# yalue/cudabrot

Measured on AMD Instinct MI355X. Metric: Msamples/sec (escaping points) + HBM GB/s, 4096x4096 max_iter=20000, 1/2/4/8 GPU, higher is better.
Workload: dtype f64

## Files before the change

cudabrot_amd/csrc/draw_wide.hip:

```cpp
#include <stdlib.h>

#include "draw_common.h"

#ifdef CB_BURNING_SHIP
#define CB_LAUNCH_NAME launch_draw_wide_ship
#else
#define CB_LAUNCH_NAME launch_draw_wide
#endif

namespace cb {

namespace {

constexpr int kWavesPerBlock = 4;
constexpr int kSlots = 4;
constexpr int kQ0Cap = 128;
constexpr int kQ1Cap = 96;
constexpr int kQ2Cap = 320;
constexpr int kHeadSteps = 4;
constexpr int kQ1Low = 32;
constexpr int kReplayMin = 56;
constexpr uint32_t kReplayBurst = 32;
constexpr int kPrioBehind = 2;
constexpr int kPrioAhead = 1;
constexpr uint32_t kBrentBits = 2;
constexpr uint32_t kPrioChunks = 64;
constexpr uint32_t kPrioHalves = 256;

static_assert(kQ0Cap >= 63 + 64, "Q0 must hold a full HEAD half-pass on top of 63 queued survivors");
static_assert(kQ1Cap >= kQ1Low - 1 + 64, "Q1 must hold a full MID pass on top of kQ1Low - 1 queued orbits");
static_assert(kQ2Cap >= 63 + 64 * kSlots, "Q2 must hold every orbit slot of a chunk on top of 63 queued points");

struct WideQueues {
  double q0_cr[kQ0Cap], q0_ci[kQ0Cap];
  double q1_cr[kQ1Cap], q1_ci[kQ1Cap], q1_r[kQ1Cap], q1_i[kQ1Cap];
  double q2_cr[kQ2Cap], q2_ci[kQ2Cap];
};
constexpr uint32_t kWideQueueWords = sizeof(WideQueues) / 8;
constexpr uint32_t kWideLanePlanes = kSlots * 6 + 2 + 4 + 1;
constexpr uint32_t kWidePlanesFront = (kCarryWordsPerWave - kCarryHeaderWords - kWideQueueWords) / 64;
__host__ __device__ constexpr uint32_t wide_plane(uint32_t p) {
  return p < kWidePlanesFront ? kCarryHeaderWords + kWideQueueWords + 64u * p
                              : kCarryWordsPerWave + kCarryHeaderWords + 64u * (p - kWidePlanesFront);
}
static_assert(kCarryHeaderWords + kWideQueueWords <= kCarryWordsPerWave, "the queues end in front of the second header");
// ... 643 lines not shown
  "v_cmpx_gt_u32_e32 vcc, %[nn], %[pidx]\n\t"    \
  "v_add_u32 %[pidx], %[q2h], %[pidx]\n\t"       \
  "v_subrev_u32 %[e], 320, %[pidx]\n\t"                   \
  "v_min_u32 %[pidx], %[pidx], %[e]\n\t"                  \
  "v_lshl_add_u32 %[pidx], %[pidx], 3, %[q2]\n\t"         \
  "ds_read_b64 %[cr], %[pidx]\n\t"                        \
  "ds_read_b64 %[ci], %[pidx] offset:2560\n\t"            \
  "s_or_b64 %[act], %[act], exec\n\t"                     \
  "v_mov_b32 %[pst], %[clk]\n\t"                          \
  "s_waitcnt lgkmcnt(0)\n\t"                              \
  "v_mul_f64 %[a], %[ci], %[ci]\n\t"             \
  "v_fma_f64 %[a], %[cr], %[cr], -%[a]\n\t"               \
  "v_fma_f64 %[i], " CB_AL "%[cr]" CB_AR ", " CB_AL "%[ci]" CB_AR ", %[ci]\n\t" \
  "v_fma_f64 %[r], %[a], 0.5, %[cr]\n\t"                  \
  "6:\n\t"                                                \
  "s_bcnt1_i32_b64 %[t], %[act]\n\t"                      \
  "s_cmp_eq_u32 %[t], 0\n\t"                              \
  "s_cbranch_scc1 2f\n\t"                                 \
  "s_sub_u32 %[ctr], %[q2c], %[nn]\n\t"          \
  "s_cmp_lg_u32 %[ctr], 0\n\t"                          \
  "s_cselect_b32 %[ctr], 1, %[minact]\n\t"              \
  "s_cmp_ge_u32 %[t], %[ctr]\n\t"                       \
  "s_cbranch_scc0 2f\n\t"
#define CBW_REPLAY_HEAD                                   \
  "s_sub_u32 %[ctr], %[n], 1\n\t"        \
  "s_mov_b32 %[ch], %[fill]\n\t"         \
  "s_mov_b64 exec, %[act]\n\t"                            \
  "v_mul_f64 %[a], %[r], %[r]\n\t"       \
  "v_fma_f64 %[a], %[i], %[i], %[a]\n\t"                  \
  "s_cmp_lg_u32 %[direct], 0\n\t"                         \
  "s_cbranch_scc1 7f\n\t"                                 \
  "1:\n\t"                                                \
  "s_bcnt1_i32_b64 %[t], %[act]\n\t"
#define CBW_REPLAY_STEP_COMMON                            \
  "s_add_u32 %[cs], %[cs], %[t]\n\t"                      \
  "v_cmp_nlt_f64_e64 %[alive], %[k16], %[a]\n\t"          \
  "v_mul_f64 %[a], %[i], %[i]\n\t"                        \
  "v_cmp_gt_u64_e64 %[hx], %[wb], %[fx]\n\t"              \
  "v_fma_f64 %[a], %[r], %[r], -%[a]\n\t"                 \
  "v_cmp_gt_u64_e64 vcc, %[hb], %[fy]\n\t"                \
  "v_fma_f64 %[i], " CB_AL "%[r]" CB_AR ", " CB_AL "%[i]" CB_AR ", %[ci]\n\t" \
  "v_cvt_i32_f64 %[col], %[fx]\n\t"                       \
  "v_fma_f64 %[r], %[a], 0.5, %[cr]\n\t"                  \
  "v_cvt_i32_f64 %[row], %[fy]\n\t"
#define CBW_REPLAY_LOOP                                   \
  CBW_REPLAY_STEP_COMMON                                  \
  "s_and_b64 vcc, vcc, %[hx]\n\t"                         \
  "v_mul_f64 %[a], %[r], %[r]\n\t"                        \
  "v_lshl_or_b32 %[e], %[row], 16, %[col]\n\t"            \
  "v_mbcnt_lo_u32_b32 %[pidx], vcc_lo, 0\n\t"             \
  "v_fma_f64 %[a], %[i], %[i], %[a]\n\t"                  \
  "v_mbcnt_hi_u32_b32 %[pidx], vcc_hi, %[pidx]\n\t"       \
  "s_bcnt1_i32_b64 %[t], vcc\n\t"                         \
  "v_add_lshl_u32 %[pidx], %[pidx], %[fill], 2\n\t"       \
  "s_and_b64 %[act], %[act], %[alive]\n\t"                \
  "s_mov_b64 exec, vcc\n\t"                               \
  "global_store_dword %[pidx], %[e], %[base]\n\t"         \
  "s_add_u32 %[fill], %[fill], %[t]\n\t"                  \
  "s_mov_b64 exec, %[act]\n\t"                            \
  "s_cbranch_execz 8f\n\t"               \
  "s_sub_u32 %[ctr], %[ctr], 1\n\t"      \
  "s_cbranch_scc0 1b\n\t"                                 \
  "s_add_u32 %[clk], %[clk], %[n]\n\t"   \
  "s_branch 18f\n\t"                                      \
  "8:\n\t"                                                \
  "s_sub_u32 %[t], %[n], %[ctr]\n\t"     \
  "s_add_u32 %[clk], %[clk], %[t]\n\t"                    \
  "18:\n\t"                                               \
  "s_sub_u32 %[ch], %[fill], %[ch]\n\t"
#define CBW_REPLAY_LOOP_CHUNKED                           \
  "s_add_u32 %[cs], %[cs], %[t]\n\t"                      \
  "v_cmp_nlt_f64_e64 %[alive], %[k16], %[a]\n\t"          \
  "v_cmp_gt_u64_e64 %[hx], %[wb], %[fx]\n\t"              \
  "v_cmp_gt_u64_e64 vcc, %[hb], %[fy]\n\t"                \
  "v_cvt_i32_f64 %[col], %[fx]\n\t"                       \
  "v_cvt_i32_f64 %[row], %[fy]\n\t"                       \
  "v_mul_f64 %[a], %[i], %[i]\n\t"                        \
  "v_mov_b32 %[lim], 1\n\t"                               \
  "s_and_b64 vcc, vcc, %[hx]\n\t"                         \
  "v_lshl_or_b32 %[e], %[row], 16, %[col]\n\t"            \
  "s_mov_b64 %[hit], vcc\n\t"                             \
  "s_mov_b64 exec, vcc\n\t"                               \
  "v_lshrrev_b32 %[row], 7, %[row]\n\t"                   \
  "v_lshrrev_b32 %[col], 7, %[col]\n\t"                   \
  "v_mad_u32_u24 %[row], %[row], %[tlx], %[col]\n\t"      \
  "v_lshrrev_b32 %[pidx], 10, %[row]\n\t"                 \
  "v_lshl_add_u32 %[col], %[pidx], 3, %[gcl]\n\t"         \
  "ds_add_rtn_u32 %[pos], %[col], %[lim]\n\t"             \
  "ds_read_b32 %[lim], %[col] offset:4\n\t"               \
  "s_bcnt1_i32_b64 %[t], vcc\n\t"                         \
  "s_mov_b64 exec, %[act]\n\t"                            \
  "v_fma_f64 %[a], %[r], %[r], -%[a]\n\t"                 \
// ... 53 lines not shown
  "s_add_u32 %[clk], %[clk], %[t]\n\t"                    \
  "9:\n\t"
#define CBW_REPLAY_END                                    \
  "2:\n\t"                                                \
  "s_mov_b64 exec, %[save]\n\t"                           \
  "s_nop 4\n\t"

struct ChunkOverflow {
  unsigned long long over;
  uint32_t word, group, pos, lim;
};
template <bool kPow2, bool kChunked>
__device__ __forceinline__ uint32_t replay_stage(uint32_t enable, unsigned long long &act, uint32_t q2_head,
                                                 uint32_t q2_count, uint32_t q2_lds, uint32_t min_active,
                                                 uint32_t n_steps, uint32_t direct, Orbit &p, uint32_t &p_start,
                                                 uint32_t *region, uint32_t &fill, uint32_t &clock,
                                                 uint32_t &lane_steps, uint32_t &hits, uint32_t cursors_lds,
                                                 ChunkOverflow &ovf) {
  static_assert(kQ2Cap == 320, "ring length and plane distance in CBW_REPLAY_REFILL");
  unsigned long long save, alive, hx, scp;
  uint32_t cs, ch, ctr, t, nn;
  double a, fx, fy, d0, d1, d2, d3, ox, oy;
  uint32_t pidx, e, col, row;
  unsigned long long over = 0ull, hit;
  uint32_t pos = 0u, lim = 0u;
  const uint32_t tlx = kChunked ? kernel_args()->bin.tiles_x : 0u;
  cursors_lds = __builtin_amdgcn_readfirstlane(cursors_lds);
  const KernelArgs ka = kernel_args();
  const double wb = ka->replay_bound_w, hb = ka->replay_bound_h;
  const uint32_t wi = (uint32_t) ka->w;
  const unsigned long long hist = reinterpret_cast<unsigned long long>(ka->hist);
  region = reinterpret_cast<uint32_t *>(uniform_u64(reinterpret_cast<unsigned long long>(region)));
  enable = __builtin_amdgcn_readfirstlane(enable);
  act = uniform_u64(act);
  fill = __builtin_amdgcn_readfirstlane(fill);
  clock = __builtin_amdgcn_readfirstlane(clock);
  n_steps = __builtin_amdgcn_readfirstlane(n_steps);
  q2_head = __builtin_amdgcn_readfirstlane(q2_head);
  q2_count = __builtin_amdgcn_readfirstlane(q2_count);
  min_active = __builtin_amdgcn_readfirstlane(min_active);
  direct = __builtin_amdgcn_readfirstlane(direct);
  const double k16 = 16.0;
  const double sx = ka->replay_scale_real, sy = ka->replay_scale_imag;
  const double oxs = ka->replay_offset_real, oys = ka->replay_offset_imag;
#define CBW_REPLAY_OUT                                                                                             \
  [r] "+v"(p.r), [i] "+v"(p.i), [cr] "+v"(p.cr), [ci] "+v"(p.ci), [pst] "+v"(p_start), [act] "+s"(act),            \
      [fill] "+s"(fill), [clk] "+s"(clock), [save] "=&s"(save), [alive] "=&s"(alive), [hx] "=&s"(hx),              \
      [cs] "=&s"(cs), [ch] "=&s"(ch), [ctr] "=&s"(ctr), [t] "=&s"(t), [nn] "=&s"(nn), [a] "=&v"(a), [fx] "=&v"(fx), \
      [fy] "=&v"(fy), [e] "=&v"(e), [col] "=&v"(col), [row] "=&v"(row), [pidx] "=&v"(pidx)
#define CBW_REPLAY_IN                                                                                              \
  [en] "s"(enable), [n] "s"(n_steps), [q2h] "s"(q2_head), [q2c] "s"(q2_count), [q2] "s"(q2_lds),                   \
      [minact] "s"(min_active), [direct] "s"(direct), [sx] "s"(sx), [sy] "s"(sy), [wb] "s"(wb), [hb] "s"(hb),      \
      [wi] "s"(wi), [hist] "s"(hist), [base] "s"(region), [k16] "s"(k16)
  (void) ox;
  (void) oy;
#define CBW_CHUNKED_OUT [over] "+s"(over), [hit] "=&s"(hit), [pos] "+v"(pos), [lim] "+v"(lim)
#define CBW_CHUNKED_IN [tlx] "s"(tlx), [gcl] "s"(cursors_lds)
  if (kPow2 && kChunked) {
    asm volatile("v_mov_b64 %[ox], %[oxs]\n\t"
                 "v_mov_b64 %[oy], %[oys]\n\t"
                 CBW_REPLAY_REFILL CBW_REPLAY_HEAD CBW_REPLAY_BIN_POW2 CBW_REPLAY_LOOP_CHUNKED
                 CBW_REPLAY_DIRECT(CBW_REPLAY_BIN_POW2) CBW_REPLAY_END
                 : CBW_REPLAY_OUT, [ox] "=&v"(ox), [oy] "=&v"(oy), CBW_CHUNKED_OUT
                 : CBW_REPLAY_IN, [oxs] "s"(oxs), [oys] "s"(oys), CBW_CHUNKED_IN
                 : "vcc", "scc", "memory");
  } else if (kPow2) {
    asm volatile("v_mov_b64 %[ox], %[oxs]\n\t"
                 "v_mov_b64 %[oy], %[oys]\n\t"
                 CBW_REPLAY_REFILL CBW_REPLAY_HEAD CBW_REPLAY_BIN_POW2 CBW_REPLAY_LOOP
                 CBW_REPLAY_DIRECT(CBW_REPLAY_BIN_POW2) CBW_REPLAY_END
                 : CBW_REPLAY_OUT, [ox] "=&v"(ox), [oy] "=&v"(oy)
                 : CBW_REPLAY_IN, [oxs] "s"(oxs), [oys] "s"(oys)
                 : "vcc", "scc", "memory");
  } else if (kChunked) {
    const double rx = ka->rcp_delta_real, ry = ka->rcp_delta_imag;
    const double kg = 0.5 - 0x1p-24;
    asm volatile(CBW_REPLAY_REFILL CBW_REPLAY_HEAD CBW_REPLAY_BIN_DIV CBW_REPLAY_LOOP_CHUNKED
                 CBW_REPLAY_DIRECT(CBW_REPLAY_BIN_DIV2) CBW_REPLAY_END
                 : CBW_REPLAY_OUT, [scp] "=&s"(scp), [d0] "=&v"(d0), [d1] "=&v"(d1), [d2] "=&v"(d2), [d3] "=&v"(d3),
                   CBW_CHUNKED_OUT
                 : CBW_REPLAY_IN, [ox] "s"(oxs), [oy] "s"(oys), [rx] "s"(rx), [ry] "s"(ry), [kg] "s"(kg), CBW_CHUNKED_IN
                 : "vcc", "scc", "memory");
  } else {
    const double rx = ka->rcp_delta_real, ry = ka->rcp_delta_imag;
    const double kg = 0.5 - 0x1p-24;
    asm volatile(CBW_REPLAY_REFILL CBW_REPLAY_HEAD CBW_REPLAY_BIN_DIV CBW_REPLAY_LOOP
                 CBW_REPLAY_DIRECT(CBW_REPLAY_BIN_DIV2) CBW_REPLAY_END
                 : CBW_REPLAY_OUT, [scp] "=&s"(scp), [d0] "=&v"(d0), [d1] "=&v"(d1), [d2] "=&v"(d2), [d3] "=&v"(d3)
                 : CBW_REPLAY_IN, [ox] "s"(oxs), [oy] "s"(oys), [rx] "s"(rx), [ry] "s"(ry), [kg] "s"(kg)
                 : "vcc", "scc", "memory");
  }
#undef CBW_CHUNKED_OUT
#undef CBW_CHUNKED_IN
  if (kChunked) {
    ovf.over = uniform_u64(over);
    ovf.word = e;
    ovf.group = pidx;
    ovf.pos = pos;
    ovf.lim = lim;
  }
#undef CBW_REPLAY_OUT
#undef CBW_REPLAY_IN
  lane_steps = cs;
  hits = ch;
  return nn;
}

__device__ __forceinline__ unsigned long long long_tail(unsigned long long mask, uint32_t n_steps, Orbit &o, int &l_rem,
                                                        uint32_t q2_tail, uint32_t q2_lds, uint32_t &lane_steps) {
  unsigned long long save, escaped;
  uint32_t cnt, tmp, ctr, slot, t;
  double a;
  const double k16 = 16.0;
// ... 412 lines not shown
    uint32_t *const st = ea->states;
    const uint32_t nt = ea->n_threads;
    const uint32_t ta = __builtin_amdgcn_readfirstlane(wave_id) * 128u + (uint32_t) lane_id();
    store_rng(st, nt, ta, rng.a);
    store_rng(st, nt, ta + 64u, rng.b);
  }
  if (kChunked) {
    const uint32_t cpw = ea->bin.chunks_per_wave;
    uint32_t *desc = ea->bin.chunk_desc + (size_t) (2u * wave_id) * cpw;
    asm volatile("" : "+s"(desc));
    const uint32_t g = (uint32_t) lane_id();
    if (g < ea->bin.n_groups) {
      const uint32_t pos = my_cursors[2u * g], lim = my_cursors[2u * g + 1u];
      if (lim != 0u) desc[lim / kChunkWords - 1u] = (g << 16) | (pos - (lim - kChunkWords));
    }
    if (lane_id() == 0) {
      uint32_t *const wc = ea->bin.wave_count;
      wc[2u * wave_id] = next_chunk < cpw ? next_chunk : cpw;
      wc[2u * wave_id + 1u] = next_chunk < cpw ? 0u : next_chunk - cpw;
    }
  } else if (lane_id() == 0) {
    uint32_t *const wc = ea->bin.wave_count;
    const uint32_t cap = ea->bin.cap;
    wc[2u * wave_id] = region_fill < cap ? region_fill : cap;
    wc[2u * wave_id + 1u] = region_fill < cap ? 0u : region_fill - cap;
  }
  {
    unsigned long long *carry = ea->carry + (size_t) wave_id * (2u * kCarryWordsPerWave);
    asm volatile("" : "+s"(carry));
    const bool holds_work = ((halves_left | pending) != 0u) || ((q0_count | q1_count | q2_count) != 0) || pact != 0ull ||
                            __ballot(l_rem[0] > 0 || l_rem[1] > 0 || l_rem[2] > 0 || l_rem[3] > 0) != 0ull;
    const unsigned long long tag = holds_work ? 2ull : 0ull;
    if (lane_id() == 0) {
      carry[0] = tag;
      carry[kCarryWordsPerWave] = tag;
      carry[1] = (unsigned long long) (uint32_t) q0_head | ((unsigned long long) (uint32_t) q0_count << 32);
      carry[2] = (unsigned long long) (uint32_t) q1_head | ((unsigned long long) (uint32_t) q1_count << 32);
      carry[3] = (unsigned long long) (uint32_t) q2_head | ((unsigned long long) (uint32_t) q2_count << 32);
      carry[4] = (unsigned long long) replay_clock;
    }
    const unsigned long long *lds_words = reinterpret_cast<const unsigned long long *>(&q);
    unsigned long long *img = carry + kCarryHeaderWords;
    for (uint32_t k = lane_id(); k < kWideQueueWords; k += 64u) img[k] = lds_words[k];
    unsigned long long *pl = carry + lane_id();
#pragma unroll
    for (int o = 0; o < kSlots; ++o) {
      pl[wide_plane(o * 6 + 0)] = (unsigned long long) __double_as_longlong(lo[o].cr);
      pl[wide_plane(o * 6 + 1)] = (unsigned long long) __double_as_longlong(lo[o].ci);
// ... 84 lines not shown
```

cudabrot_amd/csrc/kernels.h:

```cpp
#pragma once

#include <hip/hip_runtime.h>
#include <stdint.h>

#include "../../include/cudabrot_amd.h"

namespace cb {

constexpr int kSeqJumpMatrices = 64;
constexpr int kMatrixWords = 160 * 5;

void build_sequence_jump_matrices(uint32_t *out);
void seed_state(uint64_t seed, uint32_t x[5], uint32_t *d);

constexpr int kTileShift = 7;
constexpr int kTileSize = 1 << kTileShift;
constexpr int kTilePixels = kTileSize * kTileSize;
constexpr uint32_t kGroupTiles = 1024;
constexpr uint32_t kMinRegionEntries = 4096;
constexpr uint32_t kGroupReplicas = 4;
constexpr uint32_t kChunkWords = 1024;
constexpr uint32_t kRegionChunks = 32;
constexpr uint32_t kChunkedGroupsMax = 64;

struct BinLayout {
  uint32_t enabled;
  uint32_t n_waves;
  uint32_t cap;
  uint32_t n_tiles;
  uint32_t tiles_x;
  uint32_t slice_regions;
  uint32_t two_level;
  uint32_t n_groups;
  uint32_t chunked;
  uint32_t chunks_per_wave;
  uint32_t max_regions;
  uint32_t e_row_shift, e_col_mask, e_row_mask, e_chan_shift, e_chan_mask;
  uint32_t n_planes, tiles_y;
  unsigned long long plane_pixels;
  uint32_t *wave_count;
  uint32_t *stream;
  uint32_t *a_count;
  unsigned long long *a_base;
  uint32_t *grouped;
  unsigned long long *region_start;
  uint32_t *region_count;
// ... 161 lines not shown
```

cudabrot_amd/csrc/scatter.hip:

```cpp
#include <stdlib.h>
#include <string.h>

#include <type_traits>

#include "kernels.h"

namespace cb {

namespace {

constexpr int kSortPrioIo = 3;
constexpr int kSortPrioRank = 0;
constexpr int kGatherPrio = 0;
constexpr uint32_t kLeanBatch = 4;

constexpr uint32_t kScatterThreads = 512;
constexpr uint32_t kChunkEntries = 8192;
constexpr uint32_t kPerThread = kChunkEntries / kScatterThreads;
constexpr uint32_t kAccThreadsWide = 1024;
constexpr uint32_t kGroupShift = 10;
static_assert((1u << kGroupShift) == kGroupTiles, "group = tile >> kGroupShift");
constexpr uint32_t kReplicas = kGroupReplicas;
constexpr uint32_t kMaxGroups = 256;
constexpr uint32_t kMaxKeys = kMaxGroups * kGroupTiles;
constexpr uint32_t kRegionEntries = 32768;
constexpr uint32_t kSortThreads = 1024;
constexpr uint32_t kSortPerThread = kRegionEntries / kSortThreads;
constexpr uint32_t kSliceRegionsDefault = 8192;
constexpr uint32_t kGroupRegionEntries = kRegionEntries - 8u;
static_assert(kRegionEntries <= 65535, "run_start holds 16-bit positions inside a region");

size_t round_up(size_t v, size_t a) { return (v + a - 1) / a * a; }

__device__ __forceinline__ uint32_t tile_of(uint32_t e, const BinLayout &b) {
  const uint32_t plane = (e >> b.e_chan_shift) & b.e_chan_mask;
  const uint32_t tile_row = plane * b.tiles_y + (((e >> b.e_row_shift) & b.e_row_mask) >> kTileShift);
  return tile_row * b.tiles_x + ((e & b.e_col_mask) >> kTileShift);
}
__device__ __forceinline__ uint32_t offset_of(uint32_t e, const BinLayout &b) {
  return (((e >> b.e_row_shift) & b.e_row_mask & (kTileSize - 1u)) << kTileShift) |
         (e & b.e_col_mask & (kTileSize - 1u));
}
__device__ __forceinline__ void lds_inc(uint32_t *p) {
  __hip_atomic_fetch_add(p, 1u, __ATOMIC_RELAXED, __HIP_MEMORY_SCOPE_WORKGROUP);
}
__device__ __forceinline__ uint32_t wave_count_of(const BinLayout &b, uint32_t w) {
  const uint32_t n = b.wave_count[w];
  return n < b.cap ? n : b.cap;
}

__device__ __forceinline__ uint32_t block_exclusive_scan(uint32_t v, uint32_t *wave_totals,
                                                         uint32_t *total) {
  const uint32_t lane = threadIdx.x & 63u, wid = threadIdx.x >> 6;
  uint32_t inc = v;
#pragma unroll
  for (uint32_t d = 1; d < 64; d <<= 1) {
    const uint32_t up = __shfl_up(inc, d, 64);
    if (lane >= d) inc += up;
  }
  if (lane == 63u) wave_totals[wid] = inc;
  __syncthreads();
  uint32_t before = 0, all = 0;
  const uint32_t n_waves = blockDim.x >> 6;
  for (uint32_t k = 0; k < n_waves; ++k) {
    const uint32_t wt = wave_totals[k];
    if (k < wid) before += wt;
    all += wt;
  }
  *total = all;
  return before + inc - v;
}
// ... 86 lines not shown
      b.group_first[0] = 0u;
      b.group_regions[0] = total;
    }
  }
}

__global__ void __launch_bounds__(256) bin_fill_regions_kernel(BinLayout b) {
  const uint32_t r = blockIdx.x * blockDim.x + threadIdx.x;
  if (r >= *b.n_regions) return;
  uint32_t lo = 0, hi = owner_count(b);
  while (hi - lo > 1u) {
    const uint32_t mid = (lo + hi) >> 1;
    if (b.owner_first[mid] <= r) {
      lo = mid;
    } else {
      hi = mid;
    }
  }
  unsigned long long begin, entries;
  uint32_t piece;
  owner_extent(b, lo, &begin, &entries, &piece);
  const unsigned long long offset = (unsigned long long) (r - b.owner_first[lo]) * piece;
  b.region_start[r] = begin + offset;
  b.region_count[r] = (uint32_t) ((entries - offset) < piece ? (entries - offset) : piece);
  b.region_group[r] = b.two_level ? lo : 0u;
}

constexpr uint32_t kSliceTargetGroups = 12288;
constexpr uint32_t kSliceTargetGroupsTwoLevel = 6144;
static_assert(kSliceTargetGroupsTwoLevel <= kSliceTargetGroups, "the grid of the gather is sized by the larger one");
constexpr uint32_t kSliceRegionsMin = 512;
constexpr uint32_t kSliceEntriesMin = 32768;
__device__ __forceinline__ uint32_t slice_regions_for(const BinLayout &b, unsigned long long pairs,
                                                      unsigned long long entries) {
  const unsigned long long target = b.two_level ? kSliceTargetGroupsTwoLevel : kSliceTargetGroups;
  unsigned long long s = (pairs + target - 1u) / target;
  if (s < kSliceRegionsMin) s = kSliceRegionsMin;
  const unsigned long long by_entries = entries ? (kSliceEntriesMin * pairs + entries - 1u) / entries : b.slice_regions;
  if (s < by_entries) s = by_entries;
  if (s > b.slice_regions) s = b.slice_regions;
  return (uint32_t) s;
}

__global__ void __launch_bounds__(1024) bin_slice_table_kernel(BinLayout b) {
  __shared__ uint32_t wave_totals[16];
  const uint32_t nk = b.n_tiles;
  const uint32_t per = (nk + 1023u) / 1024u;
// ... 50 lines not shown
  __builtin_amdgcn_s_setprio(kSortPrioIo);
  extern __shared__ uint32_t lds[];
  uint32_t *cnt = lds + (threadIdx.x % kCntReplicas) * kCntStride;
  uint32_t *wave_totals = lds + kCntReplicas * kCntStride;
  uint2 *chunks = reinterpret_cast<uint2 *>(lds + kCntReplicas * kCntStride + 16);
  uint16_t *image = reinterpret_cast<uint16_t *>(lds + kCntReplicas * kCntStride + 16 + 2 * kRegionChunks + 4);

  const uint32_t n_regions = *b.n_regions;
  constexpr uint32_t kBatchRegions = kLean ? kRunBatch : 1u;
  for (uint32_t r_batch = blockIdx.x * kBatchRegions; r_batch < n_regions; r_batch += gridDim.x * kBatchRegions) {
  uint32_t runs[4] = {0u, 0u, 0u, 0u};
  const auto push_run = [&](uint32_t v) {
    runs[0] = __builtin_amdgcn_alignbit(runs[1], runs[0], 16);
    runs[1] = __builtin_amdgcn_alignbit(runs[2], runs[1], 16);
    runs[2] = __builtin_amdgcn_alignbit(runs[3], runs[2], 16);
    runs[3] = __builtin_amdgcn_alignbit(v, runs[3], 16);
  };
#pragma unroll 1
  for (uint32_t r = r_batch; r < r_batch + kBatchRegions; ++r) {
  if (kLean && r >= n_regions) {
    push_run(0u);
    continue;
  }
  uint32_t n = kChunked ? 0u : b.region_count[r];
  const unsigned long long start = kChunked ? (unsigned long long) r * kRegionEntries : b.region_start[r];
  const uint32_t *src = kChunked ? b.stream : (b.two_level ? b.grouped : b.stream) + start;
  const uint32_t k0 = b.region_group[r] << kGroupShift;
  const uint32_t nk = (b.n_tiles - k0) < kGroupTiles ? (b.n_tiles - k0) : kGroupTiles;
  __syncthreads();
  for (uint32_t t = threadIdx.x; t < kCntReplicas * kCntStride; t += kSortThreads) lds[t] = 0u;
  if (kChunked && threadIdx.x < 64u) {
    const uint32_t n_chunks = b.region_count[r];
    const uint2 c = threadIdx.x < n_chunks && threadIdx.x < kRegionChunks ? b.chunk_list[b.region_start[r] + threadIdx.x]
                                                                          : make_uint2(0u, 0u);
    if (threadIdx.x < kRegionChunks) chunks[threadIdx.x] = c;
    uint32_t words = c.y;
#pragma unroll
    for (uint32_t d = 32; d >= 1; d >>= 1) words += __shfl_xor(words, d, 64);
    if (threadIdx.x == 0) chunks[kRegionChunks].x = words;
  }
  __syncthreads();
  if (kChunked) n = chunks[kRegionChunks].x;

  const bool lean_region = kPlain && n != 0u && (kChunked || (start & 7ull) == 0ull);
  if (!kLean && skip_lean != 0u && lean_region) continue;
  if (kLean && !lean_region) {
    push_run(0u);
    continue;
  }
  if constexpr (kLean) {
    typedef __attribute__((address_space(3))) uint32_t *LdsWord;
    typedef __attribute__((address_space(3))) uint16_t *LdsHalf;
    const uint32_t lds0 = (uint32_t) reinterpret_cast<uintptr_t>(static_cast<void *>(lds));
    const uint32_t cnt_at = lds0 + (uint32_t) ((threadIdx.x % kCntReplicas) * kCntStride * sizeof(uint32_t)) - (k0 << 2);
    const uint32_t image_at = (uint32_t) reinterpret_cast<uintptr_t>(static_cast<void *>(image));
    const uint4 *src4 = reinterpret_cast<const uint4 *>(src);
    const uint32_t tiles_x = b.tiles_x;
    constexpr uint32_t kBatch = kChunked ? 2u : kLeanBatch;
    const auto sort_region = [&](auto masked) {
    constexpr bool kMasked = decltype(masked)::value;
    const uint32_t dummy_at = lds0 + (uint32_t) (((threadIdx.x % kCntReplicas) * kCntStride + kDummyKey) * sizeof(uint32_t));
    const uint32_t last4 = (n - 1u) >> 2;
    const uint32_t slot0 = 4u * threadIdx.x;
    const uint32_t my_chunk = threadIdx.x >> 8, in_chunk = threadIdx.x & 255u;
    const uint32_t n_chunks = kChunked ? __builtin_amdgcn_readfirstlane(b.region_count[r]) : 0u;
    const auto beyond = [&](uint32_t G) {
      return kChunked ? 4u * G >= n_chunks : (kMasked && G * 4u * kSortThreads >= n);
    };
    uint32_t e[kSortPerThread];
#pragma unroll
    for (uint32_t part = 0; part < kSortPerThread / 4u / kBatch; ++part) {
      uint4 v[kBatch];
      uint32_t words_g[kBatch];
#pragma unroll
      for (uint32_t j = 0; j < kBatch; ++j) {
        const uint32_t i4 = (part * kBatch + j) * kSortThreads + threadIdx.x;
        if (kChunked) {
          const uint2 cd = chunks[4u * (part * kBatch + j) + my_chunk];
          words_g[j] = cd.y;
          v[j] = src4[(size_t) (cd.x >> 2) + in_chunk];
        } else {
          v[j] = src4[kMasked ? (i4 < last4 ? i4 : last4) : i4];
        }
      }
#pragma unroll
      for (uint32_t j = 0; j < kBatch; ++j) {
        if (beyond(part * kBatch + j)) break;
        asm volatile("" : "+v"(v[j].x), "+v"(v[j].y), "+v"(v[j].z), "+v"(v[j].w));
        const uint32_t words[4] = {v[j].x, v[j].y, v[j].z, v[j].w};
#pragma unroll
        for (uint32_t q = 0; q < 4; ++q) {
          const uint32_t w = words[q];
          const uint32_t key = __umul24(w >> (16 + kTileShift), tiles_x) + __builtin_amdgcn_ubfe(w, kTileShift, 16 - kTileShift);
          uint32_t addr = cnt_at + (key << 2);
          if (kChunked ? !(4u * in_chunk + q < words_g[j])
                       : (kMasked && !((part * kBatch + j) * 4u * kSortThreads + q + slot0 < n))) {
            addr = dummy_at;
          }
          __hip_atomic_fetch_add((LdsWord) (uintptr_t) addr, 2u, __ATOMIC_RELAXED, __HIP_MEMORY_SCOPE_WORKGROUP);
          const uint32_t off = ((w >> (16 - kTileShift)) & ((kTileSize - 1u) << kTileShift)) |
                               (w & (kChunked ? kTileSize - 1u : ~((kTileSize - 1u) << kTileShift)));
          uint32_t packed = __builtin_amdgcn_perm(addr, off, 0x05040100u);
          asm volatile("" : "+v"(packed));
          e[4u * (part * kBatch + j) + q] = packed;
        }
      }
      asm volatile("" ::: "memory");
    }
    __syncthreads();
    {
      const bool has_key = threadIdx.x < kDummyKey;
      uint32_t c[kCntReplicas], sum = 0;
#pragma unroll
      for (uint32_t k = 0; k < kCntReplicas; ++k) {
        c[k] = has_key ? lds[k * kCntStride + threadIdx.x] : 0u;
        sum += c[k];
      }
      uint32_t first = sort_exclusive_scan(sum, wave_totals);
      __syncthreads();
      push_run(first >> 1);
#pragma unroll
      for (uint32_t k = 0; k < kCntReplicas; ++k) {
        if (has_key) lds[k * kCntStride + threadIdx.x] = image_at + first;
        first += c[k];
      }
    }
    __syncthreads();
    __builtin_amdgcn_s_setprio(kSortPrioRank);
#pragma unroll
    for (uint32_t g = 0; g < kSortPerThread / 8u; ++g) {
      if (beyond(2u * g)) break;
      uint32_t pos[8];
      const uint32_t words_a = kChunked ? chunks[4u * (2u * g) + my_chunk].y : 0u;
      const uint32_t words_b = kChunked ? chunks[4u * (2u * g + 1u) + my_chunk].y : 0u;
#pragma unroll
      for (uint32_t k = 0; k < 8u; ++k) {
        if (k == 4u && beyond(2u * g + 1u)) break;
        pos[k] = __hip_atomic_fetch_add((LdsWord) (uintptr_t) (e[8u * g + k] >> 16), 2u,
                                        __ATOMIC_RELAXED, __HIP_MEMORY_SCOPE_WORKGROUP);
      }
#pragma unroll
      for (uint32_t k = 0; k < 8u; ++k) {
        const bool inside = kChunked ? 4u * in_chunk + (k & 3u) < (k < 4u ? words_a : words_b)
// ... 50 lines not shown
        lds_inc(&cnt[key < kDummyKey ? key : kDummyKey]);
      }
    }
  } else {
    const uint32_t head = (uint32_t) (start & 3ull);
    const uint4 *src4 = reinterpret_cast<const uint4 *>(src - head);
    const uint32_t lim = head + n;
    const uint32_t last4 = lim ? (lim - 1u) >> 2 : 0u;
#pragma unroll
    for (uint32_t half = 0; half < 2; ++half) {
      uint4 v[kSortPerThread / 8u];
#pragma unroll
      for (uint32_t j = 0; j < kSortPerThread / 8u; ++j) {
        const uint32_t i4 = (half * (kSortPerThread / 8u) + j) * kSortThreads + threadIdx.x;
        v[j] = src4[i4 < last4 ? i4 : last4];
      }
#pragma unroll
      for (uint32_t j = 0; j < kSortPerThread / 8u; ++j) {
        asm volatile("" : "+v"(v[j].x), "+v"(v[j].y), "+v"(v[j].z), "+v"(v[j].w));
        const uint32_t k = half * (kSortPerThread / 8u) + j;
        const uint32_t i = (k * kSortThreads + threadIdx.x) * 4u;
        const uint32_t w0 = sort_word<kPlain>(v[j].x, k0, b), w1 = sort_word<kPlain>(v[j].y, k0, b);
        const uint32_t w2 = sort_word<kPlain>(v[j].z, k0, b), w3 = sort_word<kPlain>(v[j].w, k0, b);
        e[4 * k + 0] = (i >= head && i < lim) ? w0 : ~0u;
        e[4 * k + 1] = (i + 1u >= head && i + 1u < lim) ? w1 : ~0u;
        e[4 * k + 2] = (i + 2u >= head && i + 2u < lim) ? w2 : ~0u;
        e[4 * k + 3] = (i + 3u < lim) ? w3 : ~0u;
      }
#pragma unroll
      for (uint32_t k = half * (kSortPerThread / 2u); k < (half + 1u) * (kSortPerThread / 2u); ++k) {
        const uint32_t key = e[k] >> 16;
        lds_inc(&cnt[key < kDummyKey ? key : kDummyKey]);
      }
    }
  }
  __syncthreads();
  __builtin_amdgcn_s_setprio(kSortPrioRank);
  {
    const bool has_key = threadIdx.x < kDummyKey;
    uint32_t c[kCntReplicas], sum = 0;
#pragma unroll
    for (uint32_t k = 0; k < kCntReplicas; ++k) {
      c[k] = has_key ? lds[k * kCntStride + threadIdx.x] : 0u;
      sum += c[k];
    }
    uint32_t first = sort_exclusive_scan(sum, wave_totals);
    __syncthreads();
    if (threadIdx.x < nk) b.run_start[(size_t) threadIdx.x * b.max_regions + r] = (uint16_t) first;
#pragma unroll
    for (uint32_t k = 0; k < kCntReplicas; ++k) {
      if (has_key) lds[k * kCntStride + threadIdx.x] = first;
      first += c[k];
    }
  }
  __syncthreads();
  const uint32_t shift = (uint32_t) (start & 7ull);
#pragma unroll
  for (uint32_t k = 0; k < kSortPerThread; ++k) {
    const uint32_t key = e[k] >> 16;
    const bool real = key < kDummyKey;
    const uint32_t pos = __hip_atomic_fetch_add(&cnt[real ? key : kDummyKey], 1u, __ATOMIC_RELAXED,
                                                __HIP_MEMORY_SCOPE_WORKGROUP);
    image[real ? shift + pos : kDummyPlace] = (uint16_t) e[k];
  }
  __syncthreads();
  __builtin_amdgcn_s_setprio(kSortPrioIo);
  uint16_t *dst = b.sorted + (start - shift);
  const uint32_t lo = shift, hi = shift + n;
  const uint32_t body_lo = (lo + 7u) & ~7u, body_hi = hi & ~7u;
  if (body_lo < body_hi) {
    for (uint32_t i = lo + threadIdx.x; i < body_lo; i += kSortThreads) dst[i] = image[i];
// ... 143 lines not shown
  const uint32_t nk = b.n_groups * kReplicas;
  for (uint32_t t = threadIdx.x; t < nk; t += blockDim.x) lds[t] = 0u;
  __syncthreads();
  const uint32_t n4 = n >> 2;
  const uint4 *src4 = reinterpret_cast<const uint4 *>(src);
  for (uint32_t i = threadIdx.x; i < n4; i += blockDim.x) {
    const uint4 v = src4[i];
    const uint32_t j = i << 2;
    lds_inc(&lds[group_key(b, v.x, j)]);
    lds_inc(&lds[group_key(b, v.y, j + 1u)]);
    lds_inc(&lds[group_key(b, v.z, j + 2u)]);
    lds_inc(&lds[group_key(b, v.w, j + 3u)]);
  }
  for (uint32_t i = (n4 << 2) + threadIdx.x; i < n; i += blockDim.x) lds_inc(&lds[group_key(b, src[i], i)]);
  __syncthreads();
  for (uint32_t t = threadIdx.x; t < nk; t += blockDim.x) b.a_count[(size_t) t * b.n_waves + r] = lds[t];
}

__global__ void __launch_bounds__(64) chunk_count_kernel(BinLayout b) {
  __shared__ uint32_t cnt[kChunkedGroupsMax];
  const uint32_t w = blockIdx.x;
  cnt[threadIdx.x] = 0u;
  __syncthreads();
  const uint32_t n = b.wave_count[w] < b.chunks_per_wave ? b.wave_count[w] : b.chunks_per_wave;
  const uint32_t *desc = b.chunk_desc + (size_t) w * b.chunks_per_wave;
  for (uint32_t j = threadIdx.x; j < n; j += 64u) {
    const uint32_t g = desc[j] >> 16;
    if (g < b.n_groups) lds_inc(&cnt[g]);
  }
  __syncthreads();
  if (threadIdx.x < b.n_groups) b.a_count[(size_t) threadIdx.x * b.n_waves + w] = cnt[threadIdx.x];
}

__global__ void __launch_bounds__(64) chunk_list_kernel(BinLayout b) {
  __shared__ uint32_t cnt[kChunkedGroupsMax];
  const uint32_t w = blockIdx.x;
  cnt[threadIdx.x] = 0u;
  __syncthreads();
  const uint32_t n = b.wave_count[w] < b.chunks_per_wave ? b.wave_count[w] : b.chunks_per_wave;
  const uint32_t *desc = b.chunk_desc + (size_t) w * b.chunks_per_wave;
  for (uint32_t j = threadIdx.x; j < n; j += 64u) {
    const uint32_t d = desc[j], g = d >> 16;
    if (g >= b.n_groups) continue;
    const uint32_t words = (d & 0xffffu) < kChunkWords ? (d & 0xffffu) : kChunkWords;
    const uint32_t rank = __hip_atomic_fetch_add(&cnt[g], 1u, __ATOMIC_RELAXED, __HIP_MEMORY_SCOPE_WORKGROUP);
    const unsigned long long at = b.a_base[g] + b.a_count[(size_t) g * b.n_waves + w] + rank;
    b.chunk_list[at] = make_uint2(w * b.cap + j * kChunkWords, words);
  }
}

__global__ void __launch_bounds__(256) group_scan_rows_kernel(BinLayout b) {
  __shared__ uint32_t wave_totals[4];
  const uint32_t len = b.n_waves;
  uint32_t *row = b.a_count + (size_t) blockIdx.x * b.n_waves;
  const uint32_t per = (len + blockDim.x - 1u) / blockDim.x;
  const uint32_t w0 = threadIdx.x * per;
  uint32_t sum = 0;
  for (uint32_t k = 0; k < per; ++k) {
    if (w0 + k < len) sum += row[w0 + k];
  }
  uint32_t total = 0;
  uint32_t run = block_exclusive_scan(sum, wave_totals, &total);
// ... 216 lines not shown
    b.e_row_shift = cb_;
    b.e_col_mask = (1u << cb_) - 1u;
    b.e_row_mask = (1u << rb) - 1u;
  }
  b.slice_regions = slice_regions_setting();
  b.n_waves = n_waves;
  const Shape s = shape_of(w, h, b.n_planes);
  if (!workspace || n_waves == 0 || !s.ok) return b;
  b.n_tiles = s.n_tiles;
  b.tiles_x = s.tiles_x;
  b.tiles_y = s.tiles_y;
  b.two_level = s.two_level;
  b.n_groups = s.n_groups;
  uintptr_t p = reinterpret_cast<uintptr_t>(workspace);
  const uintptr_t p_end = p + bytes;
  p = (p + 255) & ~(uintptr_t) 255;
  if (p >= p_end) return b;
  const size_t per_entry = bytes_per_entry(s);
  const unsigned long long unit = s.chunked ? kChunkWords : 8u;
  static_assert(kMinRegionEntries % kChunkWords == 0 && kChunkWords % 8u == 0, "the search moves in units");
  unsigned long long cap = (p_end - p) / (per_entry * (size_t) n_waves);
  const unsigned long long cap_limit = 0xffffffffull / n_waves;
  if (cap > cap_limit) cap = cap_limit;
  cap = cap / unit * unit;
  const auto fits = [&](unsigned long long c) {
    const uint32_t mr = max_regions_for(s, n_waves, c * n_waves);
    return p + fixed_bytes(s, n_waves, mr) + (size_t) c * n_waves * per_entry + 1024 <= p_end;
  };
  if (cap < kMinRegionEntries || !fits(kMinRegionEntries)) return b;
  if (!fits(cap)) {
    unsigned long long lo = kMinRegionEntries, hi = cap;
    while (hi - lo > unit) {
      const unsigned long long mid = (lo + (hi - lo) / 2) / unit * unit;
      if (fits(mid)) {
        lo = mid;
      } else {
        hi = mid;
      }
    }
    cap = lo;
  }
  b.cap = (uint32_t) cap;
  b.max_regions = max_regions_for(s, n_waves, cap * n_waves);
  const size_t rows = b.n_tiles < kGroupTiles ? b.n_tiles : kGroupTiles;
  b.wave_count = carve<uint32_t>(p, (size_t) n_waves * sizeof(uint32_t), sizes.wave_count);
  b.region_start = carve<unsigned long long>(p, (size_t) b.max_regions * sizeof(unsigned long long), sizes.region_start);
  b.region_count = carve<uint32_t>(p, (size_t) b.max_regions * sizeof(uint32_t), sizes.region_count);
// ... 53 lines not shown
    }
    hipLaunchKernelGGL(group_scatter_kernel, dim3(b.n_waves), dim3(kScatterThreads), scatter_lds, stream, b);
  }
  hipLaunchKernelGGL(bin_region_heads_kernel, dim3(1), dim3(1024), 0, stream, b);
  hipLaunchKernelGGL(bin_fill_regions_kernel, dim3((b.max_regions + 255u) / 256u), dim3(256), 0, stream, b);
  hipLaunchKernelGGL(bin_slice_table_kernel, dim3(1), dim3(1024), 0, stream, b);
  const bool plain = b.n_planes == 1u && b.e_row_shift == 16u && b.e_col_mask == 0xffffu && b.e_row_mask == 0xffffu &&
                     b.e_chan_mask == 0u;
  const bool few = b.n_tiles <= kFewTilesMax;
  uint32_t skip_lean = 0u;
  const auto launch_sort = [&](auto kernel, size_t lds_bytes, uint32_t batch = 1u) -> hipError_t {
    const hipError_t e = hipFuncSetAttribute(reinterpret_cast<const void *>(kernel),
                                             hipFuncAttributeMaxDynamicSharedMemorySize, (int) lds_bytes);
    if (e != hipSuccess) return e;
    const uint32_t batches = (b.max_regions + batch - 1u) / batch;
    const uint32_t grid = batches < kSortGrid ? batches : kSortGrid;
    hipLaunchKernelGGL(kernel, dim3(grid), dim3(kSortThreads), lds_bytes, stream, b, skip_lean);
    return hipSuccess;
  };
  hipError_t se;
  if (b.chunked) {
    se = plain ? launch_sort(bin_region_sort_kernel<true, false, true, true>, SortLds<false>::kBytes, kRunBatch)
               : launch_sort(bin_region_sort_kernel<false, false, true>, SortLds<false>::kBytes);
  } else if (plain && !b.two_level && b.tiles_x <= 128u) {
    se = few ? launch_sort(bin_region_sort_kernel<true, true, false, true>, SortLds<true>::kBytes, kRunBatch)
             : launch_sort(bin_region_sort_kernel<true, false, false, true>, SortLds<false>::kBytes, kRunBatch);
    if (se == hipSuccess && (b.cap & 7u) != 0u) {
      skip_lean = 1u;
      se = few ? launch_sort(bin_region_sort_kernel<true, true>, SortLds<true>::kBytes)
               : launch_sort(bin_region_sort_kernel<true, false>, SortLds<false>::kBytes);
    }
  } else if (few) {
    se = plain ? launch_sort(bin_region_sort_kernel<true, true>, SortLds<true>::kBytes)
               : launch_sort(bin_region_sort_kernel<false, true>, SortLds<true>::kBytes);
  } else {
    se = plain ? launch_sort(bin_region_sort_kernel<true, false>, SortLds<false>::kBytes)
               : launch_sort(bin_region_sort_kernel<false, false>, SortLds<false>::kBytes);
  }
  if (se != hipSuccess) return se;
  const unsigned long long rows = b.n_tiles < kGroupTiles ? b.n_tiles : kGroupTiles;
  const unsigned long long by_cap = rows * b.max_regions / b.slice_regions;
  const unsigned long long slices = b.n_tiles + (by_cap > kSliceTargetGroups ? by_cap : kSliceTargetGroups) + 1ull;
  const auto launch_gather = [&](auto kernel) {
    hipLaunchKernelGGL(kernel, dim3((uint32_t) slices), dim3(kAccThreadsWide), 0, stream, b, hist, w, h);
  };
  if (b.two_level) launch_gather(bin_gather_accumulate_kernel<kAccThreadsWide, true>);
  else launch_gather(bin_gather_accumulate_kernel<kAccThreadsWide, false>);
// ... 5 lines not shown
```

Before: 118,100.

## Batch replay histogram hits into dwordx4 block stores with sentinel padding

The replay loop no longer issues one global_store_dword per step. Each step's hit word goes into one of four reserved VGPRs, and every four steps the wave writes them as a single dwordx4 store, with -1 sentinels filling slots for lanes that missed. The region sort kernels learn a 'blocked' flag in the wave counts, clamp sentinel keys to an extra key bucket, and shrink region counts so the padding is dropped. This cuts store instruction count and per-step address math in exchange for more stream traffic from padding, four pinned VGPRs, and extra sort-side handling.

```diff
diff --git a/cudabrot_amd/csrc/draw_wide.hip b/cudabrot_amd/csrc/draw_wide.hip
--- a/cudabrot_amd/csrc/draw_wide.hip
+++ b/cudabrot_amd/csrc/draw_wide.hip
@@ -21,6 +21,7 @@
 constexpr int kQ1Low = 32;
 constexpr int kReplayMin = 56;
 constexpr uint32_t kReplayBurst = 32;
+static_assert(kReplayBurst % 4u == 0u, "a burst is whole groups of four steps (CBW_REPLAY_LOOP_BLOCKED)");
 constexpr int kPrioBehind = 2;
 constexpr int kPrioAhead = 1;
 constexpr uint32_t kBrentBits = 2;
@@ -710,7 +711,7 @@
   "s_cselect_b32 %[ctr], 1, %[minact]\n\t"              \
   "s_cmp_ge_u32 %[t], %[ctr]\n\t"                       \
   "s_cbranch_scc0 2f\n\t"
-#define CBW_REPLAY_HEAD                                   \
+#define CBW_REPLAY_HEAD(PRE)                              \
   "s_sub_u32 %[ctr], %[n], 1\n\t"        \
   "s_mov_b32 %[ch], %[fill]\n\t"         \
   "s_mov_b64 exec, %[act]\n\t"                            \
@@ -718,6 +719,7 @@
   "v_fma_f64 %[a], %[i], %[i], %[a]\n\t"                  \
   "s_cmp_lg_u32 %[direct], 0\n\t"                         \
   "s_cbranch_scc1 7f\n\t"                                 \
+  PRE                                                     \
   "1:\n\t"                                                \
   "s_bcnt1_i32_b64 %[t], %[act]\n\t"
 #define CBW_REPLAY_STEP_COMMON                            \
@@ -731,31 +733,62 @@
   "v_cvt_i32_f64 %[col], %[fx]\n\t"                       \
   "v_fma_f64 %[r], %[a], 0.5, %[cr]\n\t"                  \
   "v_cvt_i32_f64 %[row], %[fy]\n\t"
-#define CBW_REPLAY_LOOP                                   \
+#define CBW_BLOCK_FLUSH                                   \
+  "s_mov_b64 vcc, %[blk]\n\t"                             \
+  "s_mov_b64 exec, vcc\n\t"                               \
+  "s_lshr_b32 %[t], %[fill], 2\n\t"                       \
+  "v_mbcnt_lo_u32_b32 %[pidx], vcc_lo, 0\n\t"             \
+  "v_mbcnt_hi_u32_b32 %[pidx], vcc_hi, %[pidx]\n\t"       \
+  "v_add_lshl_u32 %[pidx], %[pidx], %[t], 4\n\t"          \
+  "s_bcnt1_i32_b64 %[t], vcc\n\t"                         \
+  "global_store_dwordx4 %[pidx], v[124:127], %[base]\n\t" \
+  "s_lshl_b32 %[t], %[t], 2\n\t"                          \
+  "s_add_u32 %[fill], %[fill], %[t]\n\t"                  \
+  "s_nop 1\n\t"
+#define CBW_BLOCK_CLEAR                                   \
+  "s_mov_b64 %[blk], 0\n\t"                               \
+  "s_mov_b64 exec, -1\n\t"             \
+  "v_mov_b32 v124, -1\n\t"                                \
+  "v_mov_b32 v125, -1\n\t"                                \
+  "v_mov_b32 v126, -1\n\t"                                \
+  "v_mov_b32 v127, -1\n\t"                                \
+  "s_mov_b64 exec, %[act]\n\t"
+#define CBW_BLOCK_CLOBBERS "v124", "v125", "v126", "v127"
+#define CBW_REPLAY_BLOCKED_PRE                            \
+  "s_mov_b32 %[ch], 0\n\t"                                \
+  CBW_BLOCK_CLEAR
+#define CBW_BLOCK_STEP(EJ)                                \
   CBW_REPLAY_STEP_COMMON                                  \
   "s_and_b64 vcc, vcc, %[hx]\n\t"                         \
   "v_mul_f64 %[a], %[r], %[r]\n\t"                        \
-  "v_lshl_or_b32 %[e], %[row], 16, %[col]\n\t"            \
-  "v_mbcnt_lo_u32_b32 %[pidx], vcc_lo, 0\n\t"             \
+  "s_or_b64 %[blk], %[blk], vcc\n\t"                      \
   "v_fma_f64 %[a], %[i], %[i], %[a]\n\t"                  \
-  "v_mbcnt_hi_u32_b32 %[pidx], vcc_hi, %[pidx]\n\t"       \
   "s_bcnt1_i32_b64 %[t], vcc\n\t"                         \
-  "v_add_lshl_u32 %[pidx], %[pidx], %[fill], 2\n\t"       \
   "s_and_b64 %[act], %[act], %[alive]\n\t"                \
   "s_mov_b64 exec, vcc\n\t"                               \
-  "global_store_dword %[pidx], %[e], %[base]\n\t"         \
-  "s_add_u32 %[fill], %[fill], %[t]\n\t"                  \
+  "v_lshl_or_b32 " EJ ", %[row], 16, %[col]\n\t"          \
+  "s_add_u32 %[ch], %[ch], %[t]\n\t"                      \
   "s_mov_b64 exec, %[act]\n\t"                            \
-  "s_cbranch_execz 8f\n\t"               \
-  "s_sub_u32 %[ctr], %[ctr], 1\n\t"      \
-  "s_cbranch_scc0 1b\n\t"                                 \
+  "s_cbranch_execz 8f\n\t"             \
+  "s_sub_u32 %[ctr], %[ctr], 1\n\t"    \
+  "s_cbranch_scc1 28f\n\t"
+#define CBW_BLOCK_NEXT                                    \
+  "s_bcnt1_i32_b64 %[t], %[act]\n\t"
+#define CBW_REPLAY_LOOP_BLOCKED(BIN)                      \
+  BIN CBW_BLOCK_STEP("v124")                              \
+  CBW_BLOCK_NEXT BIN CBW_BLOCK_STEP("v125")               \
+  CBW_BLOCK_NEXT BIN CBW_BLOCK_STEP("v126")               \
+  CBW_BLOCK_NEXT BIN CBW_BLOCK_STEP("v127")               \
+  CBW_BLOCK_FLUSH CBW_BLOCK_CLEAR                         \
+  "s_branch 1b\n\t"                                       \
+  "28:\n\t"                                               \
   "s_add_u32 %[clk], %[clk], %[n]\n\t"   \
   "s_branch 18f\n\t"                                      \
   "8:\n\t"                                                \
   "s_sub_u32 %[t], %[n], %[ctr]\n\t"     \
   "s_add_u32 %[clk], %[clk], %[t]\n\t"                    \
   "18:\n\t"                                               \
-  "s_sub_u32 %[ch], %[fill], %[ch]\n\t"
+  CBW_BLOCK_FLUSH
 #define CBW_REPLAY_LOOP_CHUNKED                           \
   "s_add_u32 %[cs], %[cs], %[t]\n\t"                      \
   "v_cmp_nlt_f64_e64 %[alive], %[k16], %[a]\n\t"          \
@@ -855,7 +888,7 @@
   uint32_t cs, ch, ctr, t, nn;
   double a, fx, fy, d0, d1, d2, d3, ox, oy;
   uint32_t pidx, e, col, row;
-  unsigned long long over = 0ull, hit;
+  unsigned long long over = 0ull, hit, blk;
   uint32_t pos = 0u, lim = 0u;
   const uint32_t tlx = kChunked ? kernel_args()->bin.tiles_x : 0u;
   cursors_lds = __builtin_amdgcn_readfirstlane(cursors_lds);
@@ -892,7 +925,7 @@
   if (kPow2 && kChunked) {
     asm volatile("v_mov_b64 %[ox], %[oxs]\n\t"
                  "v_mov_b64 %[oy], %[oys]\n\t"
-                 CBW_REPLAY_REFILL CBW_REPLAY_HEAD CBW_REPLAY_BIN_POW2 CBW_REPLAY_LOOP_CHUNKED
+                 CBW_REPLAY_REFILL CBW_REPLAY_HEAD("") CBW_REPLAY_BIN_POW2 CBW_REPLAY_LOOP_CHUNKED
                  CBW_REPLAY_DIRECT(CBW_REPLAY_BIN_POW2) CBW_REPLAY_END
                  : CBW_REPLAY_OUT, [ox] "=&v"(ox), [oy] "=&v"(oy), CBW_CHUNKED_OUT
                  : CBW_REPLAY_IN, [oxs] "s"(oxs), [oys] "s"(oys), CBW_CHUNKED_IN
@@ -900,15 +933,15 @@
   } else if (kPow2) {
     asm volatile("v_mov_b64 %[ox], %[oxs]\n\t"
                  "v_mov_b64 %[oy], %[oys]\n\t"
-                 CBW_REPLAY_REFILL CBW_REPLAY_HEAD CBW_REPLAY_BIN_POW2 CBW_REPLAY_LOOP
+                 CBW_REPLAY_REFILL CBW_REPLAY_HEAD(CBW_REPLAY_BLOCKED_PRE) CBW_REPLAY_LOOP_BLOCKED(CBW_REPLAY_BIN_POW2)
                  CBW_REPLAY_DIRECT(CBW_REPLAY_BIN_POW2) CBW_REPLAY_END
-                 : CBW_REPLAY_OUT, [ox] "=&v"(ox), [oy] "=&v"(oy)
+                 : CBW_REPLAY_OUT, [ox] "=&v"(ox), [oy] "=&v"(oy), [blk] "=&s"(blk)
                  : CBW_REPLAY_IN, [oxs] "s"(oxs), [oys] "s"(oys)
-                 : "vcc", "scc", "memory");
+                 : "vcc", "scc", "memory", CBW_BLOCK_CLOBBERS);
   } else if (kChunked) {
     const double rx = ka->rcp_delta_real, ry = ka->rcp_delta_imag;
     const double kg = 0.5 - 0x1p-24;
-    asm volatile(CBW_REPLAY_REFILL CBW_REPLAY_HEAD CBW_REPLAY_BIN_DIV CBW_REPLAY_LOOP_CHUNKED
+    asm volatile(CBW_REPLAY_REFILL CBW_REPLAY_HEAD("") CBW_REPLAY_BIN_DIV CBW_REPLAY_LOOP_CHUNKED
                  CBW_REPLAY_DIRECT(CBW_REPLAY_BIN_DIV2) CBW_REPLAY_END
                  : CBW_REPLAY_OUT, [scp] "=&s"(scp), [d0] "=&v"(d0), [d1] "=&v"(d1), [d2] "=&v"(d2), [d3] "=&v"(d3),
                    CBW_CHUNKED_OUT
@@ -917,11 +950,12 @@
   } else {
     const double rx = ka->rcp_delta_real, ry = ka->rcp_delta_imag;
     const double kg = 0.5 - 0x1p-24;
-    asm volatile(CBW_REPLAY_REFILL CBW_REPLAY_HEAD CBW_REPLAY_BIN_DIV CBW_REPLAY_LOOP
+    asm volatile(CBW_REPLAY_REFILL CBW_REPLAY_HEAD(CBW_REPLAY_BLOCKED_PRE) CBW_REPLAY_LOOP_BLOCKED(CBW_REPLAY_BIN_DIV)
                  CBW_REPLAY_DIRECT(CBW_REPLAY_BIN_DIV2) CBW_REPLAY_END
-                 : CBW_REPLAY_OUT, [scp] "=&s"(scp), [d0] "=&v"(d0), [d1] "=&v"(d1), [d2] "=&v"(d2), [d3] "=&v"(d3)
+                 : CBW_REPLAY_OUT, [scp] "=&s"(scp), [d0] "=&v"(d0), [d1] "=&v"(d1), [d2] "=&v"(d2), [d3] "=&v"(d3),
+                   [blk] "=&s"(blk)
                  : CBW_REPLAY_IN, [ox] "s"(oxs), [oy] "s"(oys), [rx] "s"(rx), [ry] "s"(ry), [kg] "s"(kg)
-                 : "vcc", "scc", "memory");
+                 : "vcc", "scc", "memory", CBW_BLOCK_CLOBBERS);
   }
 #undef CBW_CHUNKED_OUT
 #undef CBW_CHUNKED_IN
@@ -1380,8 +1414,8 @@
   } else if (lane_id() == 0) {
     uint32_t *const wc = ea->bin.wave_count;
     const uint32_t cap = ea->bin.cap;
-    wc[2u * wave_id] = region_fill < cap ? region_fill : cap;
-    wc[2u * wave_id + 1u] = region_fill < cap ? 0u : region_fill - cap;
+    wc[2u * wave_id] = (region_fill < cap ? region_fill : cap) | kStreamBlocked;
+    wc[2u * wave_id + 1u] = (region_fill < cap ? 0u : region_fill - cap) | kStreamBlocked;
   }
   {
     unsigned long long *carry = ea->carry + (size_t) wave_id * (2u * kCarryWordsPerWave);
diff --git a/cudabrot_amd/csrc/kernels.h b/cudabrot_amd/csrc/kernels.h
--- a/cudabrot_amd/csrc/kernels.h
+++ b/cudabrot_amd/csrc/kernels.h
@@ -22,6 +22,8 @@
 constexpr uint32_t kChunkWords = 1024;
 constexpr uint32_t kRegionChunks = 32;
 constexpr uint32_t kChunkedGroupsMax = 64;
+constexpr uint32_t kStreamBlocked = 1u << 31;
+constexpr uint32_t kStreamSentinel = 0xffffffffu;
 
 struct BinLayout {
   uint32_t enabled;
diff --git a/cudabrot_amd/csrc/scatter.hip b/cudabrot_amd/csrc/scatter.hip
--- a/cudabrot_amd/csrc/scatter.hip
+++ b/cudabrot_amd/csrc/scatter.hip
@@ -1,3 +1,4 @@
+#include <assert.h>
 #include <stdlib.h>
 #include <string.h>
 
@@ -45,8 +46,11 @@
   __hip_atomic_fetch_add(p, 1u, __ATOMIC_RELAXED, __HIP_MEMORY_SCOPE_WORKGROUP);
 }
 __device__ __forceinline__ uint32_t wave_count_of(const BinLayout &b, uint32_t w) {
-  const uint32_t n = b.wave_count[w];
+  const uint32_t n = b.wave_count[w] & ~kStreamBlocked;
   return n < b.cap ? n : b.cap;
+}
+__device__ __forceinline__ uint32_t wave_form_of(const BinLayout &b, uint32_t w) {
+  return (b.two_level || b.chunked) ? 0u : (b.wave_count[w] & kStreamBlocked);
 }
 
 __device__ __forceinline__ uint32_t block_exclusive_scan(uint32_t v, uint32_t *wave_totals,
@@ -179,7 +183,7 @@
   owner_extent(b, lo, &begin, &entries, &piece);
   const unsigned long long offset = (unsigned long long) (r - b.owner_first[lo]) * piece;
   b.region_start[r] = begin + offset;
-  b.region_count[r] = (uint32_t) ((entries - offset) < piece ? (entries - offset) : piece);
+  b.region_count[r] = (uint32_t) ((entries - offset) < piece ? (entries - offset) : piece) | wave_form_of(b, lo);
   b.region_group[r] = b.two_level ? lo : 0u;
 }
 
@@ -276,7 +280,9 @@
     push_run(0u);
     continue;
   }
-  uint32_t n = kChunked ? 0u : b.region_count[r];
+  const uint32_t region_word = kChunked ? 0u : b.region_count[r];
+  const bool blocked = (region_word & kStreamBlocked) != 0u;
+  uint32_t n = region_word & ~kStreamBlocked;
   const unsigned long long start = kChunked ? (unsigned long long) r * kRegionEntries : b.region_start[r];
   const uint32_t *src = kChunked ? b.stream : (b.two_level ? b.grouped : b.stream) + start;
   const uint32_t k0 = b.region_group[r] << kGroupShift;
@@ -311,6 +317,7 @@
     const uint4 *src4 = reinterpret_cast<const uint4 *>(src);
     const uint32_t tiles_x = b.tiles_x;
     constexpr uint32_t kBatch = kChunked ? 2u : kLeanBatch;
+    constexpr uint32_t kSentKey = kDummyKey + 1u;
     const auto sort_region = [&](auto masked) {
     constexpr bool kMasked = decltype(masked)::value;
     const uint32_t dummy_at = lds0 + (uint32_t) (((threadIdx.x % kCntReplicas) * kCntStride + kDummyKey) * sizeof(uint32_t));
@@ -345,7 +352,8 @@
 #pragma unroll
         for (uint32_t q = 0; q < 4; ++q) {
           const uint32_t w = words[q];
-          const uint32_t key = __umul24(w >> (16 + kTileShift), tiles_x) + __builtin_amdgcn_ubfe(w, kTileShift, 16 - kTileShift);
+          uint32_t key = __umul24(w >> (16 + kTileShift), tiles_x) + __builtin_amdgcn_ubfe(w, kTileShift, 16 - kTileShift);
+          if (!kChunked) key = key < kSentKey ? key : kSentKey;
           uint32_t addr = cnt_at + (key << 2);
           if (kChunked ? !(4u * in_chunk + q < words_g[j])
                        : (kMasked && !((part * kBatch + j) * 4u * kSortThreads + q + slot0 < n))) {
@@ -373,6 +381,15 @@
       uint32_t first = sort_exclusive_scan(sum, wave_totals);
       __syncthreads();
       push_run(first >> 1);
+      if (!kChunked && blocked && threadIdx.x == kSortThreads - 1u) {
+        uint32_t at = first + sum;
+        b.region_count[r] = at >> 1;
+        for (uint32_t k = 0; k < kCntReplicas; ++k) {
+          const uint32_t c_sent = lds[k * kCntStride + kSentKey];
+          lds[k * kCntStride + kSentKey] = image_at + at;
+          at += c_sent;
+        }
+      }
 #pragma unroll
       for (uint32_t k = 0; k < kCntReplicas; ++k) {
         if (has_key) lds[k * kCntStride + threadIdx.x] = image_at + first;
@@ -469,10 +486,10 @@
         const uint32_t i = (k * kSortThreads + threadIdx.x) * 4u;
         const uint32_t w0 = sort_word<kPlain>(v[j].x, k0, b), w1 = sort_word<kPlain>(v[j].y, k0, b);
         const uint32_t w2 = sort_word<kPlain>(v[j].z, k0, b), w3 = sort_word<kPlain>(v[j].w, k0, b);
-        e[4 * k + 0] = (i >= head && i < lim) ? w0 : ~0u;
-        e[4 * k + 1] = (i + 1u >= head && i + 1u < lim) ? w1 : ~0u;
-        e[4 * k + 2] = (i + 2u >= head && i + 2u < lim) ? w2 : ~0u;
-        e[4 * k + 3] = (i + 3u < lim) ? w3 : ~0u;
+        e[4 * k + 0] = (i >= head && i < lim && !(blocked && v[j].x == kStreamSentinel)) ? w0 : ~0u;
+        e[4 * k + 1] = (i + 1u >= head && i + 1u < lim && !(blocked && v[j].y == kStreamSentinel)) ? w1 : ~0u;
+        e[4 * k + 2] = (i + 2u >= head && i + 2u < lim && !(blocked && v[j].z == kStreamSentinel)) ? w2 : ~0u;
+        e[4 * k + 3] = (i + 3u < lim && !(blocked && v[j].w == kStreamSentinel)) ? w3 : ~0u;
       }
 #pragma unroll
       for (uint32_t k = half * (kSortPerThread / 2u); k < (half + 1u) * (kSortPerThread / 2u); ++k) {
@@ -494,6 +511,7 @@
     uint32_t first = sort_exclusive_scan(sum, wave_totals);
     __syncthreads();
     if (threadIdx.x < nk) b.run_start[(size_t) threadIdx.x * b.max_regions + r] = (uint16_t) first;
+    if (blocked && threadIdx.x == kSortThreads - 1u) b.region_count[r] = first + sum;
 #pragma unroll
     for (uint32_t k = 0; k < kCntReplicas; ++k) {
       if (has_key) lds[k * kCntStride + threadIdx.x] = first;
@@ -683,7 +701,7 @@
   const uint32_t w = blockIdx.x;
   cnt[threadIdx.x] = 0u;
   __syncthreads();
-  const uint32_t n = b.wave_count[w] < b.chunks_per_wave ? b.wave_count[w] : b.chunks_per_wave;
+  const uint32_t n = wave_count_of(b, w) < b.chunks_per_wave ? wave_count_of(b, w) : b.chunks_per_wave;
   const uint32_t *desc = b.chunk_desc + (size_t) w * b.chunks_per_wave;
   for (uint32_t j = threadIdx.x; j < n; j += 64u) {
     const uint32_t g = desc[j] >> 16;
@@ -698,7 +716,7 @@
   const uint32_t w = blockIdx.x;
   cnt[threadIdx.x] = 0u;
   __syncthreads();
-  const uint32_t n = b.wave_count[w] < b.chunks_per_wave ? b.wave_count[w] : b.chunks_per_wave;
+  const uint32_t n = wave_count_of(b, w) < b.chunks_per_wave ? wave_count_of(b, w) : b.chunks_per_wave;
   const uint32_t *desc = b.chunk_desc + (size_t) w * b.chunks_per_wave;
   for (uint32_t j = threadIdx.x; j < n; j += 64u) {
     const uint32_t d = desc[j], g = d >> 16;
@@ -961,7 +979,9 @@
   unsigned long long cap = (p_end - p) / (per_entry * (size_t) n_waves);
   const unsigned long long cap_limit = 0xffffffffull / n_waves;
   if (cap > cap_limit) cap = cap_limit;
+  if (cap >= kStreamBlocked) cap = kStreamBlocked - 1u;
   cap = cap / unit * unit;
+  assert(cap < kStreamBlocked);
   const auto fits = [&](unsigned long long c) {
     const uint32_t mr = max_regions_for(s, n_waves, c * n_waves);
     return p + fixed_bytes(s, n_waves, mr) + (size_t) c * n_waves * per_entry + 1024 <= p_end;
@@ -1061,7 +1081,7 @@
   if (b.chunked) {
     se = plain ? launch_sort(bin_region_sort_kernel<true, false, true, true>, SortLds<false>::kBytes, kRunBatch)
                : launch_sort(bin_region_sort_kernel<false, false, true>, SortLds<false>::kBytes);
-  } else if (plain && !b.two_level && b.tiles_x <= 128u) {
+  } else if (plain && !b.two_level && b.tiles_x <= 128u && (few || b.tiles_x >= 2u)) {
     se = few ? launch_sort(bin_region_sort_kernel<true, true, false, true>, SortLds<true>::kBytes, kRunBatch)
              : launch_sort(bin_region_sort_kernel<true, false, false, true>, SortLds<false>::kBytes, kRunBatch);
     if (se == hipSuccess && (b.cap & 7u) != 0u) {
```

Measured after the change: 119,900 (median of 6 runs). 1.02x the previous value.
